# beehive-lab/GPULlama3.java

Hardware: AMD Instinct MI355X
Metric: tg128 tok/s (llama-bench), Llama-3-8B Q8_0 (higher is better)
Workload: dtype i8; 1 GPU; Llama-3-8B-random Q8_0 random-weight GGUF-layout model, tg128 at depth 0 (one step = 128 decode tokens, logits D2H inside the timed region); parallelism=single GPU, ranks=1, ctx=648

## Files before the change

### gpullama3.java_amd/csrc/gl3_api.hip

```cpp
#include <chrono>
#include <cstdio>
#include <cstdlib>
#include <cstring>
#include <vector>

#include "gl3_ctx.h"
#include "gl3_batch_plan.h"
#include "gl3_decode_kernels.h"
#include "gl3_rowlane_kernels.h"
#include "gl3_veclane_kernels.h"
#include "gl3_moe_kernels.h"
#include "gl3_kv_copy.h"

using namespace gl3;

static std::string g_create_err;

static double now_ms() {
    return std::chrono::duration<double, std::milli>(std::chrono::steady_clock::now().time_since_epoch()).count();
}


static int q8_tile_groups(int k) { return ((k / 32) + 3) / 4; }
static size_t matvec_smem(int pro, int epi, int k) {
    const int nm = epi == EPI_SWIGLU ? 2 : 1, ng = q8_tile_groups(k);
    return (size_t)ng * 4 * 32 + (size_t)ng * 4 * 4 + (pro == PRO_RMS ? (size_t)(k + 32) * 4 : 0) + (size_t)2 * nm * ng * 64 * 4 + 128;
}
constexpr size_t GL3_LDS_MAX = 160 * 1024 - 256;

#include <hip/hip_ext.h>
using MvKernel = void (*)(const MatvecArgs);
static void launch_mv(gl3_ctx* ctx, MvKernel kernel, dim3 grid, int threads, size_t smem, const MatvecArgs& a) {
    if (ctx->prof_ev0) hipExtLaunchKernelGGL(kernel, grid, dim3(threads), (uint32_t)smem, ctx->stream, ctx->prof_ev0, ctx->prof_ev1, 0, a);
    else hipLaunchKernelGGL(kernel, grid, dim3(threads), smem, ctx->stream, a);
}

struct MvVariant { int pro, epi, npw; bool sel, tpf, segs; MvKernel kernel; };
template <int PRO, int EPI, int NPW, bool SEL, bool TPF, bool SEGS>
constexpr MvVariant mv_variant() { return {PRO, EPI, NPW, SEL, TPF, SEGS, matvec_q8t_kernel<PRO, EPI, NPW, SEL, TPF, SEGS>}; }
constexpr MvVariant MV_VARIANTS[] = {
    mv_variant<PRO_RMS,   EPI_STORE,  4, false, false, false>(),
    mv_variant<PRO_RMS,   EPI_STORE,  4, false, false, true>(),
    mv_variant<PRO_RMS,   EPI_STORE,  4, false, true,  false>(),
    mv_variant<PRO_RMS,   EPI_STORE,  4, false, true,  true>(),
    mv_variant<PRO_RMS,   EPI_SWIGLU, 4, false, false, false>(),
    mv_variant<PRO_RMS,   EPI_SWIGLU, 4, false, false, true>(),
    mv_variant<PRO_RMS,   EPI_SWIGLU, 4, false, true,  false>(),
    mv_variant<PRO_RMS,   EPI_SWIGLU, 4, false, true,  true>(),
    mv_variant<PRO_QUANT, EPI_RESID,  4, false, false, false>(),
    mv_variant<PRO_QUANT, EPI_RESID,  4, false, false, true>(),
    mv_variant<PRO_QUANT, EPI_RESID,  4, false, true,  false>(),
    mv_variant<PRO_QUANT, EPI_RESID,  4, false, true,  true>(),
    mv_variant<PRO_QUANT, EPI_RESID,  8, false, false, false>(),
    mv_variant<PRO_QUANT, EPI_RESID,  8, false, false, true>(),
    mv_variant<PRO_QUANT, EPI_RESID,  8, false, true,  false>(),
    mv_variant<PRO_QUANT, EPI_RESID,  8, false, true,  true>(),
    mv_variant<PRO_RMS,   EPI_SWIGLU, 4, true,  false, false>(),
    mv_variant<PRO_QUANT, EPI_RESID,  4, true,  false, false>(),
};
constexpr int mv_find(int pro, int epi, int npw, bool sel, bool tpf, bool segs) {
    int i = 0;
    for (const MvVariant& v : MV_VARIANTS) {
        if (v.pro == pro && v.epi == epi && v.npw == npw && v.sel == sel && v.tpf == tpf && v.segs == segs) return i;
        ++i;
    }
    return -1;
}
[[noreturn]] static void no_kernel(const char* what, int a, int b) { fprintf(stderr, "gl3: no %s kernel for (%d, %d)\n", what, a, b); abort(); }

static void launch_q8t(gl3_ctx* ctx, int pro, int epi, const MatvecArgs& a, int slots = 0) {
    static const int max_wgs = getenv("GL3_WGS") ? atoi(getenv("GL3_WGS")) : 512;
    const bool sel = slots > 0;
    const int npw = !sel && pro == PRO_QUANT && epi == EPI_RESID && a.nstrips <= MV_WIDE_STRIPS ? 8 : 4;
    const bool segs = !sel && a.ng > mv_seg_groups(npw, epi);
    const int i = mv_find(pro, epi, npw, sel, a.tp != nullptr, segs);
    if (i < 0) no_kernel("matvec_q8t_kernel<prologue, epilogue>", pro, epi);
    launch_mv(ctx, MV_VARIANTS[i].kernel, dim3(a.nstrips < max_wgs ? a.nstrips : max_wgs, sel ? slots : 1), mv_threads(npw), matvec_smem(pro, epi, a.k), a);
}

template <int V> using IntC = std::integral_constant<int, V>;
template <typename F>
static void wt_dispatch(int fmt, bool v512, F&& f) {
    if (fmt == GL3_TYPE_F16 && v512) f(IntC<WT_F16>{}, IntC<512>{});
    else if (fmt == GL3_TYPE_F16) f(IntC<WT_F16>{}, IntC<256>{});
    else if (fmt == GL3_FMT_Q8V) f(IntC<WT_Q8_0>{}, IntC<256>{});
    else f(IntC<WT_Q4_0>{}, IntC<256>{});
}
template <typename F>
static void epi_dispatch(int epi, F&& f) {
    if (epi == EPI_STORE) f(IntC<EPI_STORE>{}); else if (epi == EPI_RESID) f(IntC<EPI_RESID>{}); else f(IntC<EPI_SWIGLU>{});
}
using RlKernel = void (*)(const RlArgs);
static RlKernel rl_kernel(int fmt, int epi) {
    RlKernel k = nullptr;
    wt_dispatch(fmt, false, [&](auto wt, auto) { epi_dispatch(epi, [&](auto e) {
        if constexpr (decltype(wt)::value != WT_Q8_0) k = matvec_rl_kernel<decltype(wt)::value, decltype(e)::value>;
    }); });
    if (!k) no_kernel("matvec_rl_kernel<format, epilogue>", fmt, epi);
    return k;
}

static void launch_matvec(gl3_ctx* ctx, int pro, int epi, const Q8Mat& w, const Q8Mat* w2, const float* x,
                          const float* norm_w, float* out, const float* resid_in, float out_scale = 1.0f, const TpRec* tp = nullptr) {
    if (w.fmt != GL3_TYPE_Q8_0) {
        hipStream_t s = ctx->stream;
        const bool ksplit_type = w.vl && (w.fmt == GL3_FMT_Q8V || w.fmt == GL3_TYPE_Q4_0);
        const long vl_waves = (long)((w.rows + 7) / 8) * (epi == EPI_SWIGLU ? 2 : 1);
        const bool fuse_rms = pro == PRO_RMS && w.vl && vl_rms_fusable(w.k) && epi != EPI_RESID && !(ksplit_type && vl_waves <= 512);
        if (pro == PRO_RMS && !fuse_rms) {
            hipLaunchKernelGGL(rmsnorm_f32_kernel, dim3(1), dim3(256), rmsnorm_smem_bytes(w.k), s, x, w.k, norm_w, ctx->d.rms_eps, ctx->xn);
            x = ctx->xn;
        }
        if (w.vl) {
            VlArgs v{};
            v.w = w.w; v.w2 = w2 ? w2->w : nullptr; v.rows = w.rows; v.k = w.k; v.x = x; v.out = out; v.resid_in = resid_in; v.out_scale = out_scale;
            v.tp = tp;
            if (fuse_rms) { v.norm_w = norm_w; v.eps = ctx->d.rms_eps; }
            const int ngroups = (w.rows + 7) / 8;
            wt_dispatch(w.fmt, ctx->d.flags & GL3_FLAG_VECTOR_512, [&](auto wt, auto species) { epi_dispatch(epi, [&](auto e) {
                constexpr int WT = decltype(wt)::value, SPECIES = decltype(species)::value, EPI = decltype(e)::value, NM = EPI == EPI_SWIGLU ? 2 : 1;
                if constexpr (EPI != EPI_RESID)
                    if (fuse_rms) {
                        hipLaunchKernelGGL((matvec_vl_kernel<WT, EPI, true, VL_RMS_WAVES, SPECIES>), dim3((ngroups + VL_RMS_WAVES - 1) / VL_RMS_WAVES), dim3(64 * VL_RMS_WAVES),
                                           vl_rms_smem_bytes(w.k), s, v);
                        return;
                    }
                if constexpr (WT == WT_F16)
                    hipLaunchKernelGGL((matvec_vl_kernel<WT, EPI, false, VL_WAVES, SPECIES>), dim3((ngroups + VL_WAVES - 1) / VL_WAVES), dim3(64 * VL_WAVES), vl_smem_bytes(w.k), s, v);
                else {
                    const int nw = vq_waves<WT>(w.k, NM, ngroups);
// ... 1153 lines not shown
    const AttnPlan p = attn_plan(s, attn_regime(s, pos));
    *regime_out = p.regime;
    *n_launches = p.n;
    for (int i = 0; i < p.n; ++i) {
        const AttnLaunch& k = p.launch[i];
        const int64_t rec[6] = {k.kernel, k.gx, k.gy, k.block, (int64_t)k.lds, (int64_t)attn_lds_cap(k.kernel)};
        memcpy(launches_out + 6 * i, rec, sizeof(rec));
    }
    head_out[0] = (int64_t)attn_head_smem(head_size, group); head_out[1] = attn_head_admits(head_size); head_out[2] = attn_head_admits(head_size, group);
    return GL3_OK;
}

int32_t gl3_get_attn_rows(gl3_ctx* ctx, int32_t out[4]) {
    if (!ctx) return GL3_E_ARG;
    if (!out) GL3_FAIL(GL3_E_ARG, "null out");
    if (!ctx->pf) GL3_FAIL(GL3_E_UNSUPPORTED, "batched steps need max_batch > 1");
    return gl3_prefill_attn_rows(ctx, out);
}

int32_t gl3_sample_rows(gl3_ctx* ctx, const float* logits, int32_t n, const float* temperature, const float* topp, const float* coins,
                        int32_t* tokens_out) {
    if (!ctx) return GL3_E_ARG;
    if (!logits || !temperature || !topp || !coins || n <= 0) GL3_FAIL(GL3_E_ARG, "bad logits / temperature / topp / coins arrays");
    if (!tokens_out) GL3_FAIL(GL3_E_ARG, "null tokens_out");
    int32_t r = check_batch_sampler(ctx);
    if (r != GL3_OK) return r;
    if (n > ctx->d.max_batch) GL3_FAIL(GL3_E_ARG, "batch larger than max_batch");
    bool all_greedy = false;
    if ((r = gl3_sample_batch_prepare(ctx, n, temperature, topp, coins, &all_greedy)) != GL3_OK) return r;
    if ((r = gl3_decode_batch_load_logits(ctx, logits, n)) != GL3_OK) return r;
    const float* logits_dev; const int32_t* greedy;
    gl3_decode_batch_outputs(ctx, &logits_dev, &greedy);
    if (all_greedy) {
        GL3_HIP(hipMemcpyAsync(tokens_out, greedy, (size_t)n * sizeof(int32_t), hipMemcpyDeviceToHost, ctx->stream));
        GL3_HIP(hipStreamSynchronize(ctx->stream));
        return GL3_OK;
    }
    return gl3_sample_batch_finish(ctx, logits_dev, greedy, n, tokens_out);
}

int32_t gl3_get_sample_probs_row(gl3_ctx* ctx, int32_t row, float* out) {
    if (!ctx) return GL3_E_ARG;
    if (!out) GL3_FAIL(GL3_E_ARG, "null out");
    GL3_HIP(hipSetDevice(ctx->d.device));
    return gl3_sample_probs_row(ctx, row, out);
}

int32_t gl3_profile_decode(gl3_ctx* ctx, int32_t token, int32_t pos, gl3_kernel_times* out) {
    if (!ctx || !out) return GL3_E_ARG;
    memset(out, 0, sizeof(*out));
    int32_t r = set_dyn(ctx, token, pos);
    if (r != GL3_OK) return r;
    return enqueue_decode(ctx, true, out, attn_mode(ctx, pos));
}

int32_t gl3_profile_kernel(gl3_ctx* ctx, int32_t klass, int32_t iters, double* out_us, uint64_t* bytes_per_launch) {
    if (!ctx || !out_us || iters <= 0) return GL3_E_ARG;
    if (!ctx->finalized) GL3_FAIL(GL3_E_STATE, "profile before gl3_finalize");
    if (klass < GL3_K_MATVEC_QKV || klass > GL3_K_OTHER) GL3_FAIL(GL3_E_ARG, "kernel class cannot be profiled");
    GL3_HIP(hipSetDevice(ctx->d.device));
    const gl3_model_desc& d = ctx->d;
    const int rank = d.tp_rank;
    hipEvent_t e0, e1;
    GL3_HIP(hipEventCreate(&e0)); GL3_HIP(hipEventCreate(&e1));
    auto sweep = [&]() {
        const int nl = klass == GL3_K_MATVEC_LOGITS ? 1 : d.n_layers;
        for (int l = 0; l < nl; ++l) {
            gl3_layer& L = ctx->layers[l];
            switch (klass) {
            case GL3_K_MATVEC_QKV: launch_matvec(ctx, PRO_RMS, EPI_STORE, L.wqkv, nullptr, ctx->x, L.attn_norm, ctx->qkv, nullptr); break;
            case GL3_K_MATVEC_WO: launch_matvec(ctx, PRO_QUANT, EPI_RESID, L.wo, nullptr, ctx->xb, nullptr, ctx->qkv, nullptr); break;
            case GL3_K_MATVEC_GATEUP: launch_matvec(ctx, PRO_RMS, EPI_SWIGLU, L.w1, &L.w3, ctx->x, L.ffn_norm, ctx->hb + (size_t)rank * ctx->hidden_l, nullptr); break;
            case GL3_K_MATVEC_DOWN: launch_matvec(ctx, PRO_QUANT, EPI_RESID, L.w2, nullptr, ctx->hb, nullptr, ctx->qkv, nullptr); break;
            case GL3_K_ATTENTION: launch_attention(ctx, l, attn_mode(ctx, ctx->h_dyn[1])); break;
            case GL3_K_OTHER: launch_attention(ctx, l, attn_mode(ctx, ctx->h_dyn[1]) == ATT_LONG ? ATT_LONG : ATT_MID, ATTN_BEHIND_SCORES); break;
            default: launch_matvec(ctx, PRO_RMS, EPI_STORE, ctx->wcls, nullptr, ctx->x, ctx->out_norm, ctx->logits + (size_t)rank * ctx->vocab_l, nullptr); break;
            }
        }
        return nl;
    };
    struct Quiet { gl3_ctx* c; ~Quiet() { c->tp_quiet = false; } } quiet{ctx};
    ctx->tp_quiet = true;
    sweep();
    GL3_HIP(hipEventRecord(e0, ctx->stream));
    long n = 0;
    for (int i = 0; i < iters; ++i) n += sweep();
    GL3_HIP(hipEventRecord(e1, ctx->stream));
    GL3_HIP(hipEventSynchronize(e1));
    float ms = 0;
    GL3_HIP(hipEventElapsedTime(&ms, e0, e1));
    hipEventDestroy(e0); hipEventDestroy(e1);
    *out_us = (double)ms * 1e3 / (double)n;
    if (bytes_per_launch) {
        const gl3_layer& L = ctx->layers[0];
        switch (klass) {
        case GL3_K_MATVEC_QKV: *bytes_per_launch = mv_bytes(L.wqkv) + d.dim * 4; break;
        case GL3_K_MATVEC_WO: *bytes_per_launch = mv_bytes(L.wo); break;
        case GL3_K_MATVEC_GATEUP: *bytes_per_launch = mv_bytes(L.w1) + L.w3.algo_bytes() + d.dim * 4; break;
        case GL3_K_MATVEC_DOWN: *bytes_per_launch = mv_bytes(L.w2); break;
        case GL3_K_ATTENTION: case GL3_K_OTHER: *bytes_per_launch = 0; break;
        default: *bytes_per_launch = mv_bytes(ctx->wcls) + d.dim * 4; break;
        }
    }
    return GL3_OK;
}

// ... 251 lines not shown
```

### gpullama3.java_amd/csrc/gl3_decode_kernels.h

```cpp
#pragma once
#include <hip/hip_runtime.h>
#include <stdint.h>

#include "gl3_seqsum.h"

namespace gl3 {

constexpr int TILE_BYTES = 2176;
constexpr int MV_AUX = 4;
constexpr int MV_WIDE_STRIPS = 256;
__host__ __device__ constexpr int mv_threads(int npw) { return 64 * (npw + MV_AUX); }

enum { PRO_RMS = 0, PRO_QUANT = 1 };
enum { EPI_STORE = 0, EPI_RESID = 1, EPI_SWIGLU = 2 };
__host__ __device__ constexpr int mv_ch(int epi) { return epi == EPI_SWIGLU ? 4 : 8; }
__host__ __device__ constexpr int mv_seg_groups(int npw, int epi) { return npw * mv_ch(epi); }

typedef float v4f __attribute__((ext_vector_type(4)));

#ifdef GL3_MV_TIMING
__device__ long long gl3_mv_stamp[32];
#define ATT_STAMP(i) do { if (blockIdx.x == 0 && threadIdx.x == 0) gl3_mv_stamp[i] = wall_clock64(); } while (0)
#define MV_STAMP(i, cond) do { if (blockIdx.x == 0 && (cond)) gl3_mv_stamp[i] = clock64(); } while (0)
#define PV_T(...) __VA_ARGS__
constexpr int MV_WG_STAMPS = 1024;
__device__ unsigned long long gl3_mv_wg_stamp[MV_WG_STAMPS][8];
#define MV_WG_TIME(v) v = (unsigned long long)wall_clock64()
#define MV_WG_PUT(s, v, cond) do { if (blockIdx.x < MV_WG_STAMPS && blockIdx.y == 0 && (cond)) atomicMax(&gl3_mv_wg_stamp[blockIdx.x][s], v); } while (0)
#else
#define PV_T(...)
#define MV_STAMP(i, cond)
#define MV_WG_TIME(v)
#define MV_WG_PUT(s, v, cond)
#define ATT_STAMP(i)
#endif

constexpr int TPF_MAX_PEERS = 15;
struct TpWait {
    const uint32_t* flags;
    const uint32_t* step;
    uint32_t* err;
    int mul, add, tp, me;
    unsigned spin_limit;
};
struct TpPush {
    uint32_t* ticket;
    const uint32_t* step;
    int mul, add, npeers;
    long delta[TPF_MAX_PEERS];
    uint32_t* flag[TPF_MAX_PEERS];
};
struct TpRec { TpWait w; TpPush p; };

__device__ __forceinline__ void tp_wait(const TpWait& w) {
    const uint32_t need = (__hip_atomic_load(w.step, __ATOMIC_RELAXED, __HIP_MEMORY_SCOPE_AGENT) - 1u) * (uint32_t)w.mul + (uint32_t)w.add;
    const int lane = threadIdx.x & 63;
    const bool mine = lane < w.tp && lane != w.me;
    unsigned spins = 0;
    for (;;) {
        const bool ok = !mine || (int32_t)(__hip_atomic_load(w.flags + (mine ? lane : 0), __ATOMIC_RELAXED, __HIP_MEMORY_SCOPE_SYSTEM) - need) >= 0;
        if (__builtin_amdgcn_ballot_w64(!ok) == 0) break;
        __builtin_amdgcn_s_sleep(8);
        if (++spins > w.spin_limit) { if (lane == 0) __hip_atomic_store(w.err, 1u, __ATOMIC_RELAXED, __HIP_MEMORY_SCOPE_SYSTEM); break; }
    }
    __builtin_amdgcn_fence(__ATOMIC_ACQUIRE, "");
}
__device__ __forceinline__ void tp_push_store(const TpPush& p, float* own, float v) {
    for (int j = 0; j < p.npeers; ++j)
        *reinterpret_cast<float*>(reinterpret_cast<uint8_t*>(own) + p.delta[j]) = v;
// ... 110 lines not shown

__device__ __forceinline__ uint32_t quantize_quad_pack(float4 v, float& qs_out) {
    float amax = fmaxf(fmaxf(fabsf(v.x), fabsf(v.y)), fmaxf(fabsf(v.z), fabsf(v.w)));
    amax = fmaxf(amax, __builtin_bit_cast(float, __builtin_amdgcn_update_dpp(0, __builtin_bit_cast(int, amax), 0xB1, 0xf, 0xf, false)));
    amax = fmaxf(amax, __builtin_bit_cast(float, __builtin_amdgcn_update_dpp(0, __builtin_bit_cast(int, amax), 0x4E, 0xf, 0xf, false)));
    amax = fmaxf(amax, __builtin_bit_cast(float, __builtin_amdgcn_update_dpp(0, __builtin_bit_cast(int, amax), 0x141, 0xf, 0xf, false)));
    const float qs = amax / 127.0f;
    const float ainv = qs != 0.f ? 1.0f / qs : 0.f;
    const float s0 = v.x * ainv, s1 = v.y * ainv, s2 = v.z * ainv, s3 = v.w * ainv;
    const int q0 = (int)(s0 + copysignf(0.5f, s0)), q1 = (int)(s1 + copysignf(0.5f, s1));
    const int q2 = (int)(s2 + copysignf(0.5f, s2)), q3 = (int)(s3 + copysignf(0.5f, s3));
    qs_out = (float)(_Float16)qs;
    return (uint32_t)(q0 & 0xFF) | ((uint32_t)(q1 & 0xFF) << 8) | ((uint32_t)(q2 & 0xFF) << 16) | ((uint32_t)(q3 & 0xFF) << 24);
}

__device__ __forceinline__ void quantize_quad(float4 v, int qd, uint8_t* xq, float* xs) {
    float qs;
    const uint32_t packed = quantize_quad_pack(v, qs);
    *reinterpret_cast<uint32_t*>(xq + 4 * qd) = packed;
    if ((qd & 7) == 0) xs[qd >> 3] = qs;
}

__device__ __forceinline__ size_t bdq_offset(int qd, int tok, int tslots) {
    const int blk = qd >> 3, qi = qd & 7, c = qi >> 1;
    const int g = ((c & 1) << 1) | (c >> 1);
    return ((size_t)(blk >> 1) * tslots + tok) * 64 + 16 * g + 8 * (blk & 1) + 4 * (qi & 1);
}
__device__ __forceinline__ size_t bds_offset(int blk, int tok, int tslots) { return ((size_t)(blk >> 2) * tslots + tok) * 4 + (blk & 3); }

__device__ __forceinline__ int dot32(const int4& a0, const int4& a1, const int4& b0, const int4& b1) {
    int s = 0;
    s = __builtin_amdgcn_sdot4(a0.x, b0.x, s, false); s = __builtin_amdgcn_sdot4(a0.y, b0.y, s, false);
    s = __builtin_amdgcn_sdot4(a0.z, b0.z, s, false); s = __builtin_amdgcn_sdot4(a0.w, b0.w, s, false);
    s = __builtin_amdgcn_sdot4(a1.x, b1.x, s, false); s = __builtin_amdgcn_sdot4(a1.y, b1.y, s, false);
    s = __builtin_amdgcn_sdot4(a1.z, b1.z, s, false); s = __builtin_amdgcn_sdot4(a1.w, b1.w, s, false);
    return s;
}

template <bool NT>
__device__ __forceinline__ int4 ld16(const uint8_t* p) {
    typedef int v4i __attribute__((ext_vector_type(4)));
    v4i v;
    if (NT) v = __builtin_nontemporal_load(reinterpret_cast<const v4i*>(p));
    else v = *reinterpret_cast<const v4i*>(p);
    int4 r; r.x = v.x; r.y = v.y; r.z = v.z; r.w = v.w;
    return r;
}
template <bool NT>
__device__ __forceinline__ uint16_t ld2(const uint8_t* p) {
    if (NT) return __builtin_nontemporal_load(reinterpret_cast<const uint16_t*>(p));
    return *reinterpret_cast<const uint16_t*>(p);
}

template <int PRO, int EPI, int NPW = 4, bool SEL = false, bool TPF = false, bool SEGS = false>
__global__ __launch_bounds__(mv_threads(NPW), NPW == 4 ? 4 : 2) void matvec_q8t_kernel(const MatvecArgs a_in) {
    MatvecArgs a = a_in;
    if (SEL) {
        const int slot = blockIdx.y;
        const MoeSlots m = *a.moe;
        if (slot < m.n_sel) {
            const size_t woff = (size_t)m.sel[slot] * m.sel_stride;
            a.w += woff;
            if (a.w2) a.w2 += woff;
            a.x += (size_t)slot * m.x_slot_stride;
            a.out += (size_t)slot * m.out_slot_stride;
        } else {
            const int c = slot - m.n_sel;
            const size_t woff = (size_t)c * m.sel_stride;
            a.w = m.sh_w + woff;
            a.w2 = m.sh_w2 ? m.sh_w2 + woff : nullptr;
            a.out = m.sh_out + (size_t)c * a.rows;
            const int left = m.sh_rows - c * a.rows;
            if (left < a.rows) { a.rows = left; a.nstrips = (left + 15) / 16; }
        }
    }
    constexpr int MV_PRODUCERS = NPW;
    extern __shared__ __attribute__((aligned(16))) uint8_t smem[];
    constexpr int NM = (EPI == EPI_SWIGLU) ? 2 : 1;
    constexpr int CH = mv_ch(EPI);
    const int t = threadIdx.x, lane = t & 63, wave = t >> 6;
    const int nb4 = a.ng * 4;
    constexpr int SEG = mv_seg_groups(NPW, EPI);
    const int nbatch = SEGS ? ((a.ng + NPW - 1) / NPW + CH - 1) / CH : 1;
    uint8_t* xq = smem;
    float* xs = reinterpret_cast<float*>(smem + (size_t)nb4 * 32);
    float* xf = xs + nb4;
    float* pbuf = xf + (PRO == PRO_RMS ? a.k + 32 : 0);
    float* red = pbuf + (size_t)2 * NM * a.ng * 64;
    int* sync_w = reinterpret_cast<int*>(red + 4);
    const size_t strip_bytes = (size_t)a.ng * TILE_BYTES;
    MV_STAMP(0, t == 0);
    PV_T(unsigned long long wg_t0 = 0, wg_t1 = 0, wg_t2 = 0;)
    MV_WG_TIME(wg_t0);
    if (t < 2) sync_w[t] = 0;

    if (wave < MV_PRODUCERS) {
        const int nt = (a.ng - wave + MV_PRODUCERS - 1) / MV_PRODUCERS;
        uint16_t sc[NM][CH];
        int4 lo[NM][CH], hi[NM][CH];
        auto issue = [&](int strip, int i0) {
#pragma unroll
            for (int u = 0; u < CH; ++u) {
                if (i0 + u < nt) {
                    const int g = wave + (i0 + u) * MV_PRODUCERS;
#pragma unroll
                    for (int m = 0; m < NM; ++m) {
                        const uint8_t* p = (m == 0 ? a.w : a.w2) + (size_t)strip * strip_bytes + (size_t)g * TILE_BYTES;
                        sc[m][u] = ld2<true>(p + 2 * lane);
                        lo[m][u] = ld16<true>(p + 128 + 16 * lane);
                        hi[m][u] = ld16<true>(p + 1152 + 16 * lane);
                    }
                }
            }
        };
        auto compute = [&](int i0, float* pb) {
#pragma unroll
            for (int u = 0; u < CH; ++u) {
                if (i0 + u < nt) {
                    const int g = wave + (i0 + u) * MV_PRODUCERS;
                    const int xb = 4 * g + (lane >> 4);
                    const int4 xlo = *reinterpret_cast<const int4*>(xq + 32 * xb);
                    const int4 xhi = *reinterpret_cast<const int4*>(xq + 32 * xb + 16);
                    const float xsc = xs[xb];
#pragma unroll
                    for (int m = 0; m < NM; ++m) {
                        const int isum = dot32(lo[m][u], hi[m][u], xlo, xhi);
                        pb[(size_t)m * a.ng * 64 + g * 64 + lane] = (float)isum * (h2f(sc[m][u]) * xsc);
                    }
                }
            }
        };
        int strip = blockIdx.x;
        __syncthreads();
        if (strip < a.nstrips) issue(strip, 0);
        while (__hip_atomic_load(&sync_w[1], __ATOMIC_RELAXED, __HIP_MEMORY_SCOPE_WORKGROUP) == 0) __builtin_amdgcn_s_sleep(2);
        __builtin_amdgcn_fence(__ATOMIC_ACQUIRE, "workgroup");
        MV_STAMP(3, t == 0);
        int it = 0;
        for (; strip < a.nstrips; strip += gridDim.x, ++it) {
            float* pb = pbuf + (size_t)(it & 1) * NM * a.ng * 64;
            for (int i0 = 0; i0 < nt; i0 += CH) {
                if (it != 0 || i0 != 0) issue(strip, i0);
                compute(i0, pb);
                if (SEGS) {
                    MV_STAMP(4 + 2 * it, t == 0 && it < 4 && i0 + CH >= nt);
                    MV_WG_TIME(wg_t1);
                    lds_barrier();
                }
            }
            if (SEGS) {
                for (int b = (nt + CH - 1) / CH; b < nbatch; ++b) lds_barrier();
            } else {
                MV_STAMP(4 + 2 * it, t == 0 && it < 4);
                MV_WG_TIME(wg_t1);
                __syncthreads();
            }
            MV_STAMP(5 + 2 * it, t == 0 && it < 4);
        }
        MV_WG_PUT(0, wg_t0, t == 0); MV_WG_PUT(1, wg_t1, lane == 0);
        return;
    }

    __builtin_amdgcn_s_setprio(3);
    const int ta = t - 64 * MV_PRODUCERS;
    const int nquads = a.k >> 2;
    float scale = 1.0f;
    constexpr int NXV = (PRO == PRO_RMS) ? 5 : 14;
    float4 nwv[5], xv[NXV];
    if (!TPF) {
#pragma unroll
        for (int i = 0; i < NXV; ++i) xv[i] = *reinterpret_cast<const float4*>(a.x + 4 * min(ta + 256 * i, nquads - 1));
    }
    if (PRO == PRO_RMS) {
#pragma unroll
        for (int i = 0; i < 5; ++i) nwv[i] = *reinterpret_cast<const float4*>(a.norm_w + 4 * min(ta + 256 * i, nquads - 1));
    }
    __syncthreads();
    if (TPF) {
        if (a.tp->w.flags) tp_wait(a.tp->w);
#pragma unroll
        for (int i = 0; i < NXV; ++i) xv[i] = *reinterpret_cast<const float4*>(a.x + 4 * min(ta + 256 * i, nquads - 1));
    }
    SubBarrier aux_sync{&sync_w[0], MV_AUX, 0};
    for (int b = (a.k >> 5) + ta; b < nb4; b += 256) {
        xs[b] = 0.f;
        const int4 z = {0, 0, 0, 0};
        *reinterpret_cast<int4*>(xq + 32 * b) = z;
        *reinterpret_cast<int4*>(xq + 32 * b + 16) = z;
    }
    if (PRO == PRO_RMS) {
        if (nquads <= NXV * 256) {
#pragma unroll
            for (int i = 0; i < NXV; ++i) { const int qd = ta + 256 * i; if (qd < nquads) *reinterpret_cast<float4*>(xf + 4 * qd) = xv[i]; }
        } else {
            for (int qd = ta; qd < nquads; qd += 256)
                *reinterpret_cast<float4*>(xf + 4 * qd) = *reinterpret_cast<const float4*>(a.x + 4 * qd);
        }
        if (ta < 32) xf[a.k + ta] = 0.f;
        aux_sync();
        MV_STAMP(1, ta == 0);
        float ss;
        if ((size_t)2 * NM * a.ng * 64 * 4 >= ss_scratch_bytes(a.k) && a.k >= 1024 && a.k <= 5120) {
            ss = exact_sumsq_lds(xf, a.k, reinterpret_cast<uint8_t*>(pbuf), ta, aux_sync);
        } else {
            if (wave == MV_PRODUCERS) {
                const float s1 = seq_sum_lds<true>(xf, a.k);
                if (lane == 0) red[0] = s1;
            }
            aux_sync();
            ss = red[0];
        }
        MV_STAMP(2, ta == 0);
// ... 204 lines not shown
```

### gpullama3.java_amd/hip.py

```python
from __future__ import annotations

import ctypes as C
import os

_DIR = os.path.dirname(os.path.abspath(__file__))
SO_PATH = os.environ.get("GL3_LIB") or os.path.join(_DIR, "libgpullama_hip.so")

GL3_OK = 0
E_ARG, E_UNSUPPORTED, E_OOM, E_HIP, E_RCCL, E_STATE = -1, -2, -3, -4, -5, -6
ERR_NAMES = {0: "GL3_OK", -1: "GL3_E_ARG", -2: "GL3_E_UNSUPPORTED", -3: "GL3_E_OOM", -4: "GL3_E_HIP", -5: "GL3_E_RCCL",
             -6: "GL3_E_STATE"}
FLAG_NO_GRAPH, FLAG_LAYER_TAPS, FLAG_FORCE_RCCL, FLAG_SCALAR_DOT, FLAG_F32_ACTIVATION = 1, 2, 4, 8, 16
FLAG_VECTOR_512, FLAG_VECTOR_128 = 32, 64
K_NAMES = ["matvec_qkv", "matvec_wo", "matvec_gateup", "matvec_down", "matvec_logits", "attention", "other", "collective"]

T_IDS = {"token_embd.weight": 0, "output_norm.weight": 1, "output.weight": 2, "attn_norm.weight": 3,
         "attn_q.weight": 4, "attn_k.weight": 5, "attn_v.weight": 6, "attn_output.weight": 7,
         "ffn_norm.weight": 8, "ffn_gate.weight": 9, "ffn_down.weight": 10, "ffn_up.weight": 11,
         "attn_q_norm.weight": 12, "attn_k_norm.weight": 13, "attn_q.bias": 14, "attn_k.bias": 15, "attn_v.bias": 16,
         "attn_qkv.weight": 17,
         "ffn_gate_inp.weight": 19, "ffn_gate_exps.weight": 20, "ffn_up_exps.weight": 21, "ffn_down_exps.weight": 22,
         "ffn_gate_inp_shexp.weight": 23, "ffn_gate_shexp.weight": 9, "ffn_down_shexp.weight": 10, "ffn_up_shexp.weight": 11}
T_W13 = 18

# ... 16 lines not shown
    "gl3_version": (C.c_char_p, []),
    "gl3_create": (C.c_int32, [C.POINTER(ModelDesc), C.POINTER(C.c_void_p)]),
    "gl3_upload_tensor": (C.c_int32, [C.c_void_p, C.c_int32, C.c_int32, C.c_void_p, C.c_uint64, C.c_int32]),
    "gl3_upload_rope": (C.c_int32, [C.c_void_p, C.c_void_p, C.c_void_p, C.c_uint64]),
    "gl3_tp_peer_access": (C.c_int32, [C.c_int32, C.c_void_p, C.c_int32, C.POINTER(C.c_int32)]),
    "gl3_tp_p2p_handle": (C.c_int32, [C.c_void_p, C.c_void_p, C.c_uint64]),
    "gl3_tp_p2p_attach": (C.c_int32, [C.c_void_p, C.c_void_p, C.c_uint64]),
    "gl3_tp_unique_id": (C.c_int32, [C.c_void_p, C.c_uint64]),
    "gl3_tp_init": (C.c_int32, [C.c_void_p, C.c_void_p, C.c_uint64]),
    "gl3_local_group_create": (C.c_int32, [C.c_int32, C.POINTER(C.c_void_p)]),
    "gl3_local_group_destroy": (None, [C.c_void_p]),
    "gl3_tp_attach_local": (C.c_int32, [C.c_void_p, C.c_void_p]),
    "gl3_finalize": (C.c_int32, [C.c_void_p]),
    "gl3_forward_decode": (C.c_int32, [C.c_void_p, C.c_int32, C.c_int32, C.c_void_p, C.c_void_p]),
    "gl3_forward_decode_sample": (C.c_int32, [C.c_void_p, C.c_int32, C.c_int32, C.c_float, C.c_float, C.c_float, C.POINTER(C.c_int32)]),
    "gl3_get_sample_probs": (C.c_int32, [C.c_void_p, C.c_void_p]),
    "gl3_get_topp_counts": (C.c_int32, [C.c_void_p, C.POINTER(C.c_int64), C.POINTER(C.c_int64)]),
    "gl3_tp_fold_mode": (C.c_int32, [C.c_void_p, C.POINTER(C.c_int32), C.POINTER(C.c_int32)]),
    "gl3_tp_pool_stats": (C.c_int32, [C.c_int32, C.POINTER(C.c_uint64), C.POINTER(C.c_uint64)]),
    "gl3_tp_pool_trim": (C.c_int32, [C.c_int32]),
    "gl3_pin_host_buffer": (C.c_int32, [C.c_void_p, C.c_void_p, C.c_uint64]),
    "gl3_unpin_host_buffer": (C.c_int32, [C.c_void_p, C.c_void_p]),
    "gl3_forward_prefill": (C.c_int32, [C.c_void_p, C.c_void_p, C.c_int32, C.c_int32]),
    "gl3_forward_prefill_seq": (C.c_int32, [C.c_void_p, C.c_int32, C.c_void_p, C.c_int32, C.c_int32]),
    "gl3_forward_decode_batch": (C.c_int32, [C.c_void_p, C.c_void_p, C.c_void_p, C.c_void_p, C.c_int32, C.c_void_p, C.c_void_p]),
    "gl3_forward_decode_batch_sample": (C.c_int32, [C.c_void_p, C.c_void_p, C.c_void_p, C.c_void_p, C.c_int32, C.c_void_p, C.c_void_p, C.c_void_p, C.c_void_p]),
    "gl3_forward_batch": (C.c_int32, [C.c_void_p, C.c_void_p, C.c_void_p, C.c_void_p, C.c_void_p, C.c_int32, C.c_void_p, C.c_void_p]),
    "gl3_forward_batch_sample": (C.c_int32, [C.c_void_p, C.c_void_p, C.c_void_p, C.c_void_p, C.c_void_p, C.c_int32, C.c_void_p, C.c_void_p, C.c_void_p,
                                             C.c_void_p]),
    "gl3_forward_batch_score": (C.c_int32, [C.c_void_p, C.c_void_p, C.c_void_p, C.c_void_p, C.c_void_p, C.c_int32, C.c_void_p, C.c_void_p, C.c_void_p,
                                            C.c_void_p]),
    "gl3_score_rows": (C.c_int32, [C.c_void_p, C.c_void_p, C.c_int32, C.c_void_p, C.c_void_p, C.c_void_p]),
    "gl3_forward_batch_verify": (C.c_int32, [C.c_void_p, C.c_void_p, C.c_void_p, C.c_void_p, C.c_int32, C.c_void_p, C.c_void_p, C.c_void_p,
                                             C.POINTER(C.c_int32)]),
    "gl3_verify_rows": (C.c_int32, [C.c_void_p, C.c_void_p, C.c_void_p, C.c_void_p, C.c_int32, C.c_void_p, C.c_void_p, C.c_void_p]),
    "gl3_debug_batch_plan": (C.c_int32, [C.c_void_p, C.c_void_p, C.c_void_p, C.c_int32, C.c_int32, C.c_int32, C.c_int32, C.c_void_p,
                                         C.POINTER(C.c_int32), C.c_void_p, C.POINTER(C.c_int32), C.c_void_p, C.POINTER(C.c_int32)]),
    "gl3_debug_batch_plan_split": (C.c_int32, [C.c_void_p, C.c_void_p, C.c_int32, C.c_int32, C.c_int32, C.c_int32, C.c_int32, C.c_void_p,
                                               C.POINTER(C.c_int32), C.c_void_p, C.POINTER(C.c_int32), C.c_void_p, C.POINTER(C.c_int32)]),
    "gl3_debug_decode_attn_plan": (C.c_int32, [C.c_int32] * 10 + [C.POINTER(C.c_int32), C.c_void_p, C.POINTER(C.c_int32), C.c_void_p]),
    "gl3_kv_seq_copy": (C.c_int32, [C.c_void_p, C.c_int32, C.c_void_p, C.c_int32, C.c_int32, C.c_int32]),
    "gl3_get_attn_rows": (C.c_int32, [C.c_void_p, C.c_void_p]),
    "gl3_get_sample_probs_row": (C.c_int32, [C.c_void_p, C.c_int32, C.c_void_p]),
    "gl3_sample_rows": (C.c_int32, [C.c_void_p, C.c_void_p, C.c_int32, C.c_void_p, C.c_void_p, C.c_void_p, C.c_void_p]),
    "gl3_get_kv_seq": (C.c_int32, [C.c_void_p, C.c_int32, C.c_int32, C.c_int32, C.c_void_p, C.c_void_p]),
    "gl3_get_x": (C.c_int32, [C.c_void_p, C.c_void_p]),
    "gl3_get_layer_x": (C.c_int32, [C.c_void_p, C.c_int32, C.c_void_p]),
    "gl3_get_kv": (C.c_int32, [C.c_void_p, C.c_int32, C.c_int32, C.c_void_p, C.c_void_p]),
    "gl3_get_buffer": (C.c_int32, [C.c_void_p, C.c_int32, C.c_void_p, C.c_uint64]),
    "gl3_debug_sumsq": (C.c_int32, [C.c_int32, C.c_void_p, C.c_int32, C.c_void_p]),
    "gl3_reset_kv": (C.c_int32, [C.c_void_p]),
    "gl3_profile_decode": (C.c_int32, [C.c_void_p, C.c_int32, C.c_int32, C.POINTER(KernelTimes)]),
    "gl3_profile_kernel": (C.c_int32, [C.c_void_p, C.c_int32, C.c_int32, C.POINTER(C.c_double), C.POINTER(C.c_uint64)]),
    "gl3_profile_prefill_kernel": (C.c_int32, [C.c_void_p, C.c_int32, C.c_int32, C.c_int32, C.POINTER(C.c_double), C.POINTER(C.c_uint64)]),
    "gl3_probe_peaks": (C.c_int32, [C.c_int32, C.POINTER(C.c_double), C.POINTER(C.c_double), C.POINTER(C.c_double)]),
    "gl3_get_init_ms": (C.c_int32, [C.c_void_p, C.POINTER(C.c_double), C.POINTER(C.c_double)]),
    "gl3_destroy": (None, [C.c_void_p]),
    "gl3_last_error": (C.c_char_p, [C.c_void_p]),
    "gl3_gguf_open": (C.c_int32, [C.c_char_p, C.POINTER(C.c_void_p)]),
    "gl3_gguf_close": (None, [C.c_void_p]),
    "gl3_gguf_last_error": (C.c_char_p, [C.c_void_p]),
    "gl3_gguf_tensor_count": (C.c_int32, [C.c_void_p]),
    "gl3_gguf_tensor_info": (C.c_int32, [C.c_void_p, C.c_int32, C.POINTER(C.c_char_p), C.POINTER(C.c_int32), C.POINTER(C.c_uint64),
                                         C.POINTER(C.c_void_p), C.POINTER(C.c_uint64)]),
    "gl3_gguf_meta_number": (C.c_int32, [C.c_void_p, C.c_char_p, C.POINTER(C.c_double)]),
    "gl3_gguf_meta_string": (C.c_int32, [C.c_void_p, C.c_char_p, C.POINTER(C.c_char_p)]),
    "gl3_gguf_model_desc": (C.c_int32, [C.c_void_p, C.POINTER(ModelDesc), C.POINTER(C.c_float)]),
    "gl3_rope_table": (None, [C.c_int32, C.c_int32, C.c_float, C.c_void_p, C.c_void_p]),
    "gl3_rope_table_yarn": (None, [C.c_int32, C.c_int32, C.c_float, C.c_float, C.c_float, C.c_float, C.c_float, C.c_int32,
                                   C.c_void_p, C.c_void_p]),
    "gl3_gguf_yarn_params": (C.c_int32, [C.c_void_p, C.POINTER(C.c_float), C.POINTER(C.c_float), C.POINTER(C.c_float),
                                         C.POINTER(C.c_float), C.POINTER(C.c_int32)]),
    "gl3_kquant_to_q8_0": (C.c_int32, [C.c_int32, C.c_void_p, C.c_uint64, C.c_void_p]),
    "gl3_load_gguf": (C.c_int32, [C.c_char_p, C.POINTER(ModelDesc), C.POINTER(C.c_void_p)]),
}

_lib = None


class Gl3Error(RuntimeError):
    def __init__(self, code, msg):
        super().__init__("%s (%d): %s" % (ERR_NAMES.get(code, "GL3_E_?"), code, msg))
        self.code = code


def lib():
    global _lib
    if _lib is None:
        if not os.path.exists(SO_PATH):
            raise ImportError("libgpullama_hip.so is not built: run `python __graft_entry__.py` (hipcc --offload-arch=gfx950); "
                              "there is no CPU fallback for the HIP path")
        try:
            import torch
        except Exception:
            pass
        L = C.CDLL(SO_PATH, mode=C.RTLD_GLOBAL)
        for name, (res, args) in _SIGS.items():
            fn = getattr(L, name)
            fn.restype, fn.argtypes = res, args
        _lib = L
    return _lib


def check_gguf(code: int, g=None):
    if code != 0:
        msg = lib().gl3_gguf_last_error(g)
# ... 19 lines not shown
```

### include/gpullama3_hip.h

```cpp
#ifndef GPULLAMA3_HIP_H
#define GPULLAMA3_HIP_H

#include <stddef.h>
#include <stdint.h>

#ifdef __cplusplus
extern "C" {
#endif

#define GL3_API __attribute__((visibility("default")))

typedef struct gl3_ctx gl3_ctx;

typedef enum {
    GL3_OK = 0,
    GL3_E_ARG = -1,
    GL3_E_UNSUPPORTED = -2,
    GL3_E_OOM = -3,
    GL3_E_HIP = -4,
    GL3_E_RCCL = -5,
    GL3_E_STATE = -6
} gl3_status;

enum { GL3_ARCH_LLAMA = 0, GL3_ARCH_QWEN3 = 1, GL3_ARCH_QWEN2 = 2,
// ... 115 lines not shown
                                         int32_t n, float* logits_out, int32_t* argmax_out);

GL3_API int32_t gl3_forward_decode_batch_sample(gl3_ctx* ctx, const int32_t* tokens, const int32_t* seq_ids,
                                                const int32_t* positions, int32_t n, const float* temperature,
                                                const float* topp, const float* coins, int32_t* tokens_out);
GL3_API int32_t gl3_forward_batch(gl3_ctx* ctx, const int32_t* tokens, const int32_t* seq_ids, const int32_t* positions,
                                  const int8_t* want_logits, int32_t n, float* logits_out, int32_t* argmax_out);
GL3_API int32_t gl3_forward_batch_sample(gl3_ctx* ctx, const int32_t* tokens, const int32_t* seq_ids, const int32_t* positions,
                                         const int8_t* want_logits, int32_t n, const float* temperature, const float* topp,
                                         const float* coins, int32_t* tokens_out);
typedef struct { float prob, logit, max, sum; } gl3_token_score;
GL3_API int32_t gl3_forward_batch_score(gl3_ctx* ctx, const int32_t* tokens, const int32_t* seq_ids, const int32_t* positions,
                                        const int8_t* want_logits, int32_t n, const int32_t* targets, const float* temperature,
                                        gl3_token_score* scores_out, int32_t* argmax_out);
GL3_API int32_t gl3_score_rows(gl3_ctx* ctx, const float* logits, int32_t n, const int32_t* targets, const float* temperature,
                               gl3_token_score* scores_out);
typedef struct { int32_t accepted, token; } gl3_verify_result;
GL3_API int32_t gl3_forward_batch_verify(gl3_ctx* ctx, const int32_t* tokens, const int32_t* seq_ids, const int32_t* positions, int32_t n,
                                         const float* temperature, const float* coins, gl3_verify_result* results_out,
                                         int32_t* n_runs_out);
GL3_API int32_t gl3_verify_rows(gl3_ctx* ctx, const float* logits, const int32_t* tokens, const int32_t* run_rows, int32_t n_runs,
                                const float* temperature, const float* coins, gl3_verify_result* results_out);
GL3_API int32_t gl3_debug_batch_plan(const int32_t* seq_ids, const int32_t* positions, const int8_t* want_logits, int32_t n,
                                     int32_t n_seqs, int32_t ctx, int32_t capacity, int32_t* runs_out, int32_t* n_runs,
                                     int32_t* tiles_out, int32_t* n_tiles, int32_t* out_rows, int32_t* n_out);
GL3_API int32_t gl3_debug_batch_plan_split(const int32_t* seq_ids, const int32_t* positions, int32_t n, int32_t n_seqs, int32_t ctx,
                                           int32_t capacity, int32_t fused_max_pos, int32_t* shallow_out, int32_t* n_shallow,
                                           int32_t* deep_out, int32_t* n_deep, int32_t* deep_rows, int32_t* n_deep_rows);
GL3_API int32_t gl3_debug_decode_attn_plan(int32_t head_size, int32_t kvmul, int32_t heads_l, int32_t kv_heads_l, int32_t ctx, int32_t window,
                                           int32_t attn_mid, int32_t head_kernel_allowed, int32_t pos, int32_t group, int32_t* regime_out,
                                           int64_t* launches_out, int32_t* n_launches, int64_t* head_out);
GL3_API int32_t gl3_kv_seq_copy(gl3_ctx* ctx, int32_t src_seq, const int32_t* dst_seqs, int32_t n_dst, int32_t p0, int32_t p1);
GL3_API int32_t gl3_get_attn_rows(gl3_ctx* ctx, int32_t out[4]);

GL3_API int32_t gl3_get_sample_probs_row(gl3_ctx* ctx, int32_t row, float* out);
GL3_API int32_t gl3_sample_rows(gl3_ctx* ctx, const float* logits, int32_t n, const float* temperature, const float* topp,
                                const float* coins, int32_t* tokens_out);

GL3_API int32_t gl3_get_x(gl3_ctx* ctx, float* out );
GL3_API int32_t gl3_get_layer_x(gl3_ctx* ctx, int32_t layer, float* out );
GL3_API int32_t gl3_get_kv(gl3_ctx* ctx, int32_t layer, int32_t position, float* k_out, float* v_out );
GL3_API int32_t gl3_get_kv_seq(gl3_ctx* ctx, int32_t seq, int32_t layer, int32_t position, float* k_out, float* v_out);

GL3_API int32_t gl3_get_buffer(gl3_ctx* ctx, int32_t which, float* out, uint64_t n_floats);

GL3_API int32_t gl3_debug_sumsq(int32_t device, const float* x, int32_t n, float* out);

GL3_API int32_t gl3_reset_kv(gl3_ctx* ctx);

GL3_API int32_t gl3_profile_decode(gl3_ctx* ctx, int32_t token, int32_t position, gl3_kernel_times* out);

GL3_API int32_t gl3_profile_kernel(gl3_ctx* ctx, int32_t klass, int32_t iters, double* out_us, uint64_t* bytes_per_launch);

GL3_API int32_t gl3_profile_prefill_kernel(gl3_ctx* ctx, int32_t klass, int32_t n_tokens, int32_t iters, double* out_us,
                                           uint64_t* int8_ops_per_launch);

GL3_API int32_t gl3_probe_peaks(int32_t device, double* hbm_read_gbs, double* hbm_copy_gbs, double* int8_mfma_tops);

GL3_API int32_t gl3_get_init_ms(gl3_ctx* ctx, double* plan_ms, double* copy_in_ms);

GL3_API void gl3_destroy(gl3_ctx* ctx);
GL3_API const char* gl3_last_error(gl3_ctx* ctx);

typedef struct gl3_gguf gl3_gguf;
GL3_API int32_t gl3_gguf_open(const char* path, gl3_gguf** out);
GL3_API void gl3_gguf_close(gl3_gguf* g);
GL3_API const char* gl3_gguf_last_error(const gl3_gguf* g);
GL3_API int32_t gl3_gguf_tensor_count(const gl3_gguf* g);
GL3_API int32_t gl3_gguf_tensor_info(const gl3_gguf* g, int32_t i, const char** name, int32_t* type, uint64_t* ne, const void** data,
                                     uint64_t* bytes);
GL3_API int32_t gl3_gguf_meta_number(const gl3_gguf* g, const char* key, double* out);
GL3_API int32_t gl3_gguf_meta_string(const gl3_gguf* g, const char* key, const char** out);
GL3_API int32_t gl3_gguf_model_desc(gl3_gguf* g, gl3_model_desc* desc, float* rope_theta);
GL3_API void gl3_rope_table(int32_t ctx, int32_t head_size, float theta, float* cr, float* ci);
GL3_API void gl3_rope_table_yarn(int32_t ctx, int32_t head_size, float theta, float factor, float beta_fast, float beta_slow,
                                 float log_multiplier, int32_t original_ctx, float* cr, float* ci);
GL3_API int32_t gl3_gguf_yarn_params(gl3_gguf* g, float* factor, float* beta_fast, float* beta_slow, float* log_multiplier,
                                     int32_t* original_ctx);
GL3_API int32_t gl3_kquant_to_q8_0(int32_t src_type, const void* src, uint64_t n_elements, void* dst);

GL3_API int32_t gl3_load_gguf(const char* path, const gl3_model_desc* opts, gl3_ctx** out);

#ifdef __cplusplus
}
#endif
#endif
```

Baseline: 483.1 tok/s.

## Add windowed multi-segment prefetch variant for wide gate/up SwiGLU matvec

Adds a new matvec kernel variant for the RMS-prologue SwiGLU (gate/up) projection with many strips. It uses 8 producer waves and a register window holding two segments of tiles, so loads for the next segment are issued while the current one is computed, across strip boundaries. The grid is capped at the wide-strip count and launch bounds are raised to 3 workgroups per CU. This aims to hide HBM latency in the FFN gate/up matvec, at the cost of more registers per thread and fewer workgroups. A query API exposing the chosen variant is also added.

```diff
diff --git a/gpullama3.java_amd/csrc/gl3_api.hip b/gpullama3.java_amd/csrc/gl3_api.hip
--- a/gpullama3.java_amd/csrc/gl3_api.hip
+++ b/gpullama3.java_amd/csrc/gl3_api.hip
@@ -35,9 +35,11 @@
     else hipLaunchKernelGGL(kernel, grid, dim3(threads), smem, ctx->stream, a);
 }
 
-struct MvVariant { int pro, epi, npw; bool sel, tpf, segs; MvKernel kernel; };
+struct MvVariant { int pro, epi, npw; bool sel, tpf, segs; int win, sg; MvKernel kernel; };
 template <int PRO, int EPI, int NPW, bool SEL, bool TPF, bool SEGS>
-constexpr MvVariant mv_variant() { return {PRO, EPI, NPW, SEL, TPF, SEGS, matvec_q8t_kernel<PRO, EPI, NPW, SEL, TPF, SEGS>}; }
+constexpr MvVariant mv_variant() { return {PRO, EPI, NPW, SEL, TPF, SEGS, mv_ch(EPI), mv_ch(EPI), matvec_q8t_kernel<PRO, EPI, NPW, SEL, TPF, SEGS>}; }
+template <int PRO, int EPI, int NPW, int WIN, int SG>
+constexpr MvVariant mv_variant_win() { return {PRO, EPI, NPW, false, false, true, WIN, SG, matvec_q8t_kernel<PRO, EPI, NPW, false, false, true, WIN, SG>}; }
 constexpr MvVariant MV_VARIANTS[] = {
     mv_variant<PRO_RMS,   EPI_STORE,  4, false, false, false>(),
     mv_variant<PRO_RMS,   EPI_STORE,  4, false, false, true>(),
@@ -57,25 +59,32 @@
     mv_variant<PRO_QUANT, EPI_RESID,  8, false, true,  true>(),
     mv_variant<PRO_RMS,   EPI_SWIGLU, 4, true,  false, false>(),
     mv_variant<PRO_QUANT, EPI_RESID,  4, true,  false, false>(),
+    mv_variant_win<PRO_RMS, EPI_SWIGLU, 8, MV_GU_WIN, MV_GU_SG>(),
 };
-constexpr int mv_find(int pro, int epi, int npw, bool sel, bool tpf, bool segs) {
+constexpr int mv_find(int pro, int epi, int npw, bool sel, bool tpf, bool segs, bool win = false) {
     int i = 0;
     for (const MvVariant& v : MV_VARIANTS) {
-        if (v.pro == pro && v.epi == epi && v.npw == npw && v.sel == sel && v.tpf == tpf && v.segs == segs) return i;
+        if (v.pro == pro && v.epi == epi && v.npw == npw && v.sel == sel && v.tpf == tpf && v.segs == segs && (v.win != v.sg) == win) return i;
         ++i;
     }
     return -1;
 }
 [[noreturn]] static void no_kernel(const char* what, int a, int b) { fprintf(stderr, "gl3: no %s kernel for (%d, %d)\n", what, a, b); abort(); }
 
+struct MvChoice { int index, npw, wgs; bool segs, win; };
+static MvChoice mv_choose(int pro, int epi, int ng, int nstrips, bool sel, bool tpf) {
+    static const int max_wgs = getenv("GL3_WGS") ? atoi(getenv("GL3_WGS")) : 512;
+    const bool win = !sel && !tpf && pro == PRO_RMS && epi == EPI_SWIGLU && nstrips > MV_WIDE_STRIPS && ng % (8 * MV_GU_SG) == 0;
+    const int npw = win || (!sel && pro == PRO_QUANT && epi == EPI_RESID && nstrips <= MV_WIDE_STRIPS) ? 8 : 4;
+    const bool segs = win || (!sel && ng > mv_seg_groups(npw, epi));
+    const int cap = win ? MV_WIDE_STRIPS : max_wgs;
+    return {mv_find(pro, epi, npw, sel, tpf, segs, win), npw, nstrips < cap ? nstrips : cap, segs, win};
+}
 static void launch_q8t(gl3_ctx* ctx, int pro, int epi, const MatvecArgs& a, int slots = 0) {
-    static const int max_wgs = getenv("GL3_WGS") ? atoi(getenv("GL3_WGS")) : 512;
     const bool sel = slots > 0;
-    const int npw = !sel && pro == PRO_QUANT && epi == EPI_RESID && a.nstrips <= MV_WIDE_STRIPS ? 8 : 4;
-    const bool segs = !sel && a.ng > mv_seg_groups(npw, epi);
-    const int i = mv_find(pro, epi, npw, sel, a.tp != nullptr, segs);
-    if (i < 0) no_kernel("matvec_q8t_kernel<prologue, epilogue>", pro, epi);
-    launch_mv(ctx, MV_VARIANTS[i].kernel, dim3(a.nstrips < max_wgs ? a.nstrips : max_wgs, sel ? slots : 1), mv_threads(npw), matvec_smem(pro, epi, a.k), a);
+    const MvChoice c = mv_choose(pro, epi, a.ng, a.nstrips, sel, a.tp != nullptr);
+    if (c.index < 0) no_kernel("matvec_q8t_kernel<prologue, epilogue>", pro, epi);
+    launch_mv(ctx, MV_VARIANTS[c.index].kernel, dim3(c.wgs, sel ? slots : 1), mv_threads(c.npw), matvec_smem(pro, epi, a.k), a);
 }
 
 template <int V> using IntC = std::integral_constant<int, V>;
@@ -1335,6 +1344,20 @@
     int32_t r = set_dyn(ctx, token, pos);
     if (r != GL3_OK) return r;
     return enqueue_decode(ctx, true, out, attn_mode(ctx, pos));
+}
+
+int32_t gl3_mv_variant_query(int32_t prologue, int32_t epilogue, int32_t k, int32_t rows, int32_t routed_slots, int32_t tensor_parallel,
+                             int32_t* producers, int32_t* segmented, int32_t* window_tiles, int32_t* segment_tiles, int32_t* workgroups) {
+    if (k <= 0 || k % 32 || rows <= 0) return GL3_E_ARG;
+    const MvChoice c = mv_choose(prologue, epilogue, q8_tile_groups(k), (rows + 15) / 16, routed_slots > 0, tensor_parallel != 0);
+    if (c.index < 0) return GL3_E_UNSUPPORTED;
+    const MvVariant& v = MV_VARIANTS[c.index];
+    if (producers) *producers = v.npw;
+    if (segmented) *segmented = v.segs;
+    if (window_tiles) *window_tiles = v.win;
+    if (segment_tiles) *segment_tiles = v.sg;
+    if (workgroups) *workgroups = c.wgs;
+    return GL3_OK;
 }
 
 int32_t gl3_profile_kernel(gl3_ctx* ctx, int32_t klass, int32_t iters, double* out_us, uint64_t* bytes_per_launch) {
diff --git a/gpullama3.java_amd/csrc/gl3_decode_kernels.h b/gpullama3.java_amd/csrc/gl3_decode_kernels.h
--- a/gpullama3.java_amd/csrc/gl3_decode_kernels.h
+++ b/gpullama3.java_amd/csrc/gl3_decode_kernels.h
@@ -15,6 +15,7 @@
 enum { EPI_STORE = 0, EPI_RESID = 1, EPI_SWIGLU = 2 };
 __host__ __device__ constexpr int mv_ch(int epi) { return epi == EPI_SWIGLU ? 4 : 8; }
 __host__ __device__ constexpr int mv_seg_groups(int npw, int epi) { return npw * mv_ch(epi); }
+constexpr int MV_GU_WIN = 4, MV_GU_SG = 2;
 
 typedef float v4f __attribute__((ext_vector_type(4)));
 
@@ -231,8 +232,9 @@
     return *reinterpret_cast<const uint16_t*>(p);
 }
 
-template <int PRO, int EPI, int NPW = 4, bool SEL = false, bool TPF = false, bool SEGS = false>
-__global__ __launch_bounds__(mv_threads(NPW), NPW == 4 ? 4 : 2) void matvec_q8t_kernel(const MatvecArgs a_in) {
+template <int PRO, int EPI, int NPW = 4, bool SEL = false, bool TPF = false, bool SEGS = false, int WIN = mv_ch(EPI), int SG = WIN>
+__global__ __launch_bounds__(mv_threads(NPW), NPW == 4 ? 4 : WIN != SG ? 3 : 2) void matvec_q8t_kernel(const MatvecArgs a_in) {
+    static_assert(WIN % SG == 0 && (WIN == SG || SEGS), "the window holds whole segments; the windowed form hands over at segment barriers");
     MatvecArgs a = a_in;
     if (SEL) {
         const int slot = blockIdx.y;
@@ -256,10 +258,10 @@
     constexpr int MV_PRODUCERS = NPW;
     extern __shared__ __attribute__((aligned(16))) uint8_t smem[];
     constexpr int NM = (EPI == EPI_SWIGLU) ? 2 : 1;
-    constexpr int CH = mv_ch(EPI);
+    constexpr int CH = SG;
     const int t = threadIdx.x, lane = t & 63, wave = t >> 6;
     const int nb4 = a.ng * 4;
-    constexpr int SEG = mv_seg_groups(NPW, EPI);
+    constexpr int SEG = NPW * SG;
     const int nbatch = SEGS ? ((a.ng + NPW - 1) / NPW + CH - 1) / CH : 1;
     uint8_t* xq = smem;
     float* xs = reinterpret_cast<float*>(smem + (size_t)nb4 * 32);
@@ -275,9 +277,9 @@
 
     if (wave < MV_PRODUCERS) {
         const int nt = (a.ng - wave + MV_PRODUCERS - 1) / MV_PRODUCERS;
-        uint16_t sc[NM][CH];
-        int4 lo[NM][CH], hi[NM][CH];
-        auto issue = [&](int strip, int i0) {
+        uint16_t sc[NM][WIN];
+        int4 lo[NM][WIN], hi[NM][WIN];
+        auto issue = [&](int strip, int i0, int r0 = 0) {
 #pragma unroll
             for (int u = 0; u < CH; ++u) {
                 if (i0 + u < nt) {
@@ -285,14 +287,14 @@
 #pragma unroll
                     for (int m = 0; m < NM; ++m) {
                         const uint8_t* p = (m == 0 ? a.w : a.w2) + (size_t)strip * strip_bytes + (size_t)g * TILE_BYTES;
-                        sc[m][u] = ld2<true>(p + 2 * lane);
-                        lo[m][u] = ld16<true>(p + 128 + 16 * lane);
-                        hi[m][u] = ld16<true>(p + 1152 + 16 * lane);
+                        sc[m][r0 + u] = ld2<true>(p + 2 * lane);
+                        lo[m][r0 + u] = ld16<true>(p + 128 + 16 * lane);
+                        hi[m][r0 + u] = ld16<true>(p + 1152 + 16 * lane);
                     }
                 }
             }
         };
-        auto compute = [&](int i0, float* pb) {
+        auto compute = [&](int i0, float* pb, int r0 = 0) {
 #pragma unroll
             for (int u = 0; u < CH; ++u) {
                 if (i0 + u < nt) {
@@ -303,18 +305,87 @@
                     const float xsc = xs[xb];
 #pragma unroll
                     for (int m = 0; m < NM; ++m) {
-                        const int isum = dot32(lo[m][u], hi[m][u], xlo, xhi);
-                        pb[(size_t)m * a.ng * 64 + g * 64 + lane] = (float)isum * (h2f(sc[m][u]) * xsc);
+                        const int isum = dot32(lo[m][r0 + u], hi[m][r0 + u], xlo, xhi);
+                        pb[(size_t)m * a.ng * 64 + g * 64 + lane] = (float)isum * (h2f(sc[m][r0 + u]) * xsc);
                     }
                 }
             }
         };
         int strip = blockIdx.x;
+        PV_T(unsigned long long wg_t3 = 0;)
+        if constexpr (WIN != SG) {
+            constexpr int NSLOT = WIN / SG;
+            auto issue_w = [&](int strip, int i0, int r0) {
+#pragma unroll
+                for (int u = 0; u < SG; ++u) {
+                    const int g = min(wave + (i0 + u) * MV_PRODUCERS, a.ng - 1);
+#pragma unroll
+                    for (int m = 0; m < NM; ++m) {
+                        const uint8_t* p = (m == 0 ? a.w : a.w2) + (size_t)strip * strip_bytes + (size_t)g * TILE_BYTES;
+                        sc[m][r0 + u] = ld2<true>(p + 2 * lane);
+                        lo[m][r0 + u] = ld16<true>(p + 128 + 16 * lane);
+                        hi[m][r0 + u] = ld16<true>(p + 1152 + 16 * lane);
+                    }
+                }
+            };
+            const int nmine = strip < a.nstrips ? (a.nstrips - 1 - strip) / (int)gridDim.x + 1 : 0;
+            const int nseg = nmine * nbatch;
+            int si = strip, bi = 0;
+            auto issue_next = [&](int r0) {
+                issue_w(si, bi * SG, r0);
+                if (++bi == nbatch) { bi = 0; si += gridDim.x; }
+            };
+            int it = 0, b = 0;
+            auto step = [&](int r0, bool load) {
+                compute(b * SG, pbuf + (size_t)(it & 1) * NM * a.ng * 64, r0);
+                if (load) issue_next(r0);
+                MV_WG_TIME(wg_t1);
+                lds_barrier();
+                if (++b == nbatch) { b = 0; ++it; }
+            };
+            auto wait_ready = [&]() {
+                while (__hip_atomic_load(&sync_w[1], __ATOMIC_RELAXED, __HIP_MEMORY_SCOPE_WORKGROUP) == 0) __builtin_amdgcn_s_sleep(2);
+                __builtin_amdgcn_fence(__ATOMIC_ACQUIRE, "workgroup");
+            };
+            __syncthreads();
+            if (nseg < NSLOT) {
+#pragma unroll
+                for (int j = 0; j < NSLOT; ++j) if (j < nseg) issue_next(j * SG);
+                wait_ready();
+#pragma unroll
+                for (int j = 0; j < NSLOT; ++j) if (j < nseg) step(j * SG, false);
+            } else {
+#pragma unroll
+                for (int j = 0; j < NSLOT; ++j) issue_next(j * SG);
+                PV_T(asm volatile("s_waitcnt vmcnt(0)" ::: "memory"); MV_WG_TIME(wg_t2);)
+                wait_ready();
+                MV_WG_TIME(wg_t3);
+                int s = 0;
+                for (; s + 2 * NSLOT <= nseg; s += NSLOT) {
+#pragma unroll
+                    for (int j = 0; j < NSLOT; ++j) step(j * SG, true);
+                }
+                const int r = nseg - NSLOT - s;
+#pragma unroll
+                for (int R = 0; R < NSLOT; ++R) {
+                    if (r == R) {
+#pragma unroll
+                        for (int q = 0; q < R; ++q) step(q * SG, true);
+#pragma unroll
+                        for (int q = 0; q < NSLOT; ++q) step((R + q) % NSLOT * SG, false);
+                    }
+                }
+            }
+            MV_WG_PUT(0, wg_t0, t == 0); MV_WG_PUT(1, wg_t1, lane == 0); MV_WG_PUT(5, wg_t2, lane == 0); MV_WG_PUT(6, wg_t3, lane == 0);
+            return;
+        }
         __syncthreads();
         if (strip < a.nstrips) issue(strip, 0);
+        PV_T(asm volatile("s_waitcnt vmcnt(0)" ::: "memory"); MV_WG_TIME(wg_t2);)
         while (__hip_atomic_load(&sync_w[1], __ATOMIC_RELAXED, __HIP_MEMORY_SCOPE_WORKGROUP) == 0) __builtin_amdgcn_s_sleep(2);
         __builtin_amdgcn_fence(__ATOMIC_ACQUIRE, "workgroup");
         MV_STAMP(3, t == 0);
+        MV_WG_TIME(wg_t3);
         int it = 0;
         for (; strip < a.nstrips; strip += gridDim.x, ++it) {
             float* pb = pbuf + (size_t)(it & 1) * NM * a.ng * 64;
@@ -336,7 +407,7 @@
             }
             MV_STAMP(5 + 2 * it, t == 0 && it < 4);
         }
-        MV_WG_PUT(0, wg_t0, t == 0); MV_WG_PUT(1, wg_t1, lane == 0);
+        MV_WG_PUT(0, wg_t0, t == 0); MV_WG_PUT(1, wg_t1, lane == 0); MV_WG_PUT(5, wg_t2, lane == 0); MV_WG_PUT(6, wg_t3, lane == 0);
         return;
     }
 
diff --git a/gpullama3.java_amd/hip.py b/gpullama3.java_amd/hip.py
--- a/gpullama3.java_amd/hip.py
+++ b/gpullama3.java_amd/hip.py
@@ -92,6 +92,7 @@
     "gl3_reset_kv": (C.c_int32, [C.c_void_p]),
     "gl3_profile_decode": (C.c_int32, [C.c_void_p, C.c_int32, C.c_int32, C.POINTER(KernelTimes)]),
     "gl3_profile_kernel": (C.c_int32, [C.c_void_p, C.c_int32, C.c_int32, C.POINTER(C.c_double), C.POINTER(C.c_uint64)]),
+    "gl3_mv_variant_query": (C.c_int32, [C.c_int32] * 6 + [C.POINTER(C.c_int32)] * 5),
     "gl3_profile_prefill_kernel": (C.c_int32, [C.c_void_p, C.c_int32, C.c_int32, C.c_int32, C.POINTER(C.c_double), C.POINTER(C.c_uint64)]),
     "gl3_probe_peaks": (C.c_int32, [C.c_int32, C.POINTER(C.c_double), C.POINTER(C.c_double), C.POINTER(C.c_double)]),
     "gl3_get_init_ms": (C.c_int32, [C.c_void_p, C.POINTER(C.c_double), C.POINTER(C.c_double)]),
diff --git a/include/gpullama3_hip.h b/include/gpullama3_hip.h
--- a/include/gpullama3_hip.h
+++ b/include/gpullama3_hip.h
@@ -191,6 +191,9 @@
 
 GL3_API int32_t gl3_profile_kernel(gl3_ctx* ctx, int32_t klass, int32_t iters, double* out_us, uint64_t* bytes_per_launch);
 
+GL3_API int32_t gl3_mv_variant_query(int32_t prologue, int32_t epilogue, int32_t k, int32_t rows, int32_t routed_slots, int32_t tensor_parallel,
+                                     int32_t* producers, int32_t* segmented, int32_t* window_tiles, int32_t* segment_tiles, int32_t* workgroups);
+
 GL3_API int32_t gl3_profile_prefill_kernel(gl3_ctx* ctx, int32_t klass, int32_t n_tokens, int32_t iters, double* out_us,
                                            uint64_t* int8_ops_per_launch);
 
```

Result: no change. 486.1 tok/s (median of 6 runs) (+0.6%).
